# DemianMArin/HMM_Training

Measured on NVIDIA B200. Metric: baum_welch_frames_per_s_per_iter, higher is better.
Workload: dtype f64

## Files before the change

### hmm_training_b200/csrc/bw.cu

```cuda
#include <algorithm>
#include <cstdlib>
#include <functional>
#include <memory>
#include <numeric>

#include "bw_kernels.cuh"
#include "bwltr_kernels.cuh"

namespace hmmb {

__global__ void k_load_B(const double *__restrict__ B, int N, int M, double *__restrict__ Bt,
                         int32_t *__restrict__ b_has_zero) {
    const size_t w = blockIdx.y;
    for (int e = blockIdx.x * blockDim.x + threadIdx.x; e < N * M; e += gridDim.x * blockDim.x) {
        const int k = e / N, j = e - k * N;
        const double v = B[(w * N + j) * M + k];
        Bt[w * (size_t)M * N + e] = v > 0.0 ? v : 0.0;
        if (!(v > 0.0) && b_has_zero) b_has_zero[w] = 1;
    }
}
__global__ void k_load_clamped(const double *__restrict__ src, int64_t n, double *__restrict__ dst) {
    for (int64_t e = (int64_t)blockIdx.x * blockDim.x + threadIdx.x; e < n; e += (int64_t)gridDim.x * blockDim.x) {
        const double v = src[e];
        dst[e] = v > 0.0 ? v : 0.0;
// ... 1210 lines not shown
                s.d_word, s.d_foff, s.R, per_group, h->N, h->M, h->d_pi, h->d_A, h->d_Bt, h->d_spill, h->d_llseq,
                h->act_cur, h->d_flag);
    HMMB_TRY((launch_exact<SymT, false>(h)));
    HMMB_LAUNCH("bw_backward", (k_bw_bwdG<NP, SymT>), (unsigned)grid, BW_THREADS, 0, (const SymT *)s.d_obs, s.d_off, s.d_len,
                s.d_word, s.d_foff, s.R, per_group, h->N, h->M, h->d_A, h->d_Bt, h->d_spill, h->d_llseq, h->act_cur,
                h->d_accum, h->astride, h->d_flag, h->d_newflags);
    return HMMB_OK;
}

static int bwd4_warps(int M, int rep, bool bidiag, size_t smem_optin, size_t *smem) {
    int nw = bidiag ? BWD4_MAX_WARPS : 12;
    auto bytes = [&](int w) { return (size_t)M * rep * 4 * sizeof(double) + (size_t)w * M * 4 * sizeof(double) + (size_t)w * 4 * sizeof(double); };
    const size_t avail = smem_optin > 20 * 1024 ? smem_optin - 20 * 1024 : 0;
    while (nw > 1 && bytes(nw) > avail) --nw;
    *smem = bytes(nw);
    return nw;
}

template <bool BIDIAG, int MT, int REP>
static int launch_special_estep(hmmb_bw *h) {
    Ctx &c = ctx();
    SeqSet &s = h->s;
    if (s.ncta == 0) { s.pend.reset(); return HMMB_OK; }
    const size_t smem_f = (size_t)h->M * 5 * sizeof(double) + (size_t)((h->M + 15) & ~15);
    size_t smem_b = 0;
    const int bwd_threads = 32 * bwd4_warps(h->M, REP, BIDIAG, c.smem_optin, &smem_b);
    HMMB_CUDA(cudaFuncSetAttribute((k_bw_bwd4<BIDIAG, MT, REP>), cudaFuncAttributeMaxDynamicSharedMemorySize, (int)smem_b));
    const CtaWork *stage_work = s.ncta_fine > 0 ? s.d_work_fine : s.d_work;
    const int stage_ncta = s.ncta_fine > 0 ? s.ncta_fine : s.ncta;
    auto launch_range = [&](int c0, int c1) -> int {
        if (c1 <= c0) return HMMB_OK;
        HMMB_LAUNCH("bw_forward", k_bw_fwd4<BIDIAG>, (c1 - c0) * FWD4_SPLIT, BW_THREADS, smem_f, stage_work + c0, s.d_blks, (const uint4 *)s.d_obs,
                    s.d_len, h->d_pi, h->d_A, h->d_Bt, h->M, spill4(h), h->d_llseq, h->act_cur, h->d_flag,
                    h->d_allfull, FWD4_SPLIT, SYM_MASK);
        HMMB_LAUNCH("bw_backward", (k_bw_bwd4<BIDIAG, MT, REP>), c1 - c0, bwd_threads, smem_b, stage_work + c0, s.d_blks, (const uint4 *)s.d_obs,
                    s.d_len, h->d_A, h->d_Bt, h->M, spill4(h), h->d_llseq, h->act_cur, h->d_bzero,
                    h->d_allfull, h->d_partials + (size_t)c0 * h->pstride, h->pstride, h->d_flag, h->d_newflags);
        return HMMB_OK;
    };
    if (s.pend) {
        PendingPrepare &p = *s.pend;
        int bdone = 0, cdone = 0;
        cudaStream_t main_stream = c.stream;
        const bool side = p.nstage > 2;
        struct Restore { Ctx &c; cudaStream_t s; ~Restore() { c.stream = s; } } restore{c, main_stream};
        if (side) {
            cudaEvent_t fork = event_get();
            HMMB_CUDA(cudaEventRecord(fork, main_stream));
            for (auto st : c.stage_stream) HMMB_CUDA(cudaStreamWaitEvent(st, fork, 0));
            event_put(fork);
        }
        for (int j = 0; j < p.nstage; ++j) {
            if (side) c.stream = c.stage_stream[j & 1];
            HMMB_CUDA(cudaStreamWaitEvent(c.stream, p.up->ev[p.ev_index[j]], 0));
            HMMB_TRY(launch_repack_range(s, p.up->d_raw, p.idx_bytes, bdone, p.blk_end[j], s.d_bad));
            HMMB_TRY(launch_range(cdone, p.cta_end[j]));
            bdone = p.blk_end[j];
            cdone = p.cta_end[j];
        }
        c.stream = main_stream;
        if (side) {
            for (auto st : c.stage_stream) {
                cudaEvent_t join = event_get();
                HMMB_CUDA(cudaEventRecord(join, st));
                HMMB_CUDA(cudaStreamWaitEvent(main_stream, join, 0));
                event_put(join);
            }
        }
        h->check_bad = true;
        h->pend_release = std::move(s.pend);
        HMMB_TRY((launch_exact<uint16_t, true>(h)));
        HMMB_LAUNCH("bw_exact", k_bw_llstat_fix, stage_ncta, BW_THREADS, 0, stage_work, s.d_blks, h->d_llseq, h->act_cur,
                    h->d_flag, h->d_partials, h->pstride, h->M);
        h->estep_fine = s.ncta_fine > 0;
        return HMMB_OK;
    }
    h->estep_fine = false;
    HMMB_LAUNCH("bw_forward", k_bw_fwd4<BIDIAG>, (s.ncta_fwd ? s.ncta_fwd : s.ncta) * FWD4_SPLIT, BW_THREADS, smem_f,
                s.ncta_fwd ? s.d_work_fwd : s.d_work, s.d_blks, (const uint4 *)s.d_obs,
                s.d_len, h->d_pi, h->d_A, h->d_Bt, h->M, spill4(h), h->d_llseq, h->act_cur, h->d_flag,
                h->d_allfull, FWD4_SPLIT, SYM_MASK);
    HMMB_TRY((launch_exact<uint16_t, true>(h)));
    HMMB_LAUNCH("bw_backward", (k_bw_bwd4<BIDIAG, MT, REP>), s.ncta, bwd_threads, smem_b, s.d_work, s.d_blks, (const uint4 *)s.d_obs,
                s.d_len, h->d_A, h->d_Bt, h->M, spill4(h), h->d_llseq, h->act_cur, h->d_bzero,
                h->d_allfull, h->d_partials, h->pstride, h->d_flag, h->d_newflags);
    return HMMB_OK;
}

template <int NS>
static int launch_ltr_estep(hmmb_bw *h) {
    SeqSet &s = h->sl;
    if (s.ncta == 0) return HMMB_OK;
    const int M = h->M;
    const size_t smem_f = (size_t)M * NS * 8 + (size_t)M * 8 + (size_t)M * 2;
    const size_t smem_b = (size_t)M * NS * 8 + (size_t)LTR_WARPS * 32 * Ltr<NS>::ROWB + (size_t)2 * NS * 8 +
                          (size_t)LTR_WARPS * 2 * NS * 8;
    HMMB_CUDA(cudaFuncSetAttribute(k_bw_fwdL<NS>, cudaFuncAttributeMaxDynamicSharedMemorySize, (int)smem_f));
    HMMB_CUDA(cudaFuncSetAttribute(k_bw_bwdL<NS>, cudaFuncAttributeMaxDynamicSharedMemorySize, (int)smem_b));
    if (s.pend) {
        Ctx &c = ctx();
        PendingPrepare &p = *s.pend;
        int bdone = 0, cdone = 0;
        cudaStream_t main_stream = c.stream;
        const bool side = p.nstage > 2;
        struct Restore { Ctx &c; cudaStream_t s; ~Restore() { c.stream = s; } } restore{c, main_stream};
        if (side) {
            cudaEvent_t fork = event_get();
            HMMB_CUDA(cudaEventRecord(fork, main_stream));
            for (auto st : c.stage_stream) HMMB_CUDA(cudaStreamWaitEvent(st, fork, 0));
            event_put(fork);
        }
        for (int j = 0; j < p.nstage; ++j) {
            if (side) c.stream = c.stage_stream[j & 1];
            HMMB_CUDA(cudaStreamWaitEvent(c.stream, p.up->ev[p.ev_index[j]], 0));
// ... 504 lines not shown
```

### hmm_training_b200/csrc/bw4_kernels.cuh

```cuda
#pragma once

#include <type_traits>

#include "hmm_device.cuh"

namespace hmmb {

constexpr int BW_THREADS = 128;
constexpr int BW_WARPS = BW_THREADS / 32;
constexpr int SPC4 = 8;
constexpr unsigned SYM_MASK = 0x7ffu;
constexpr int SYM_BITS = 11;
constexpr int BW4_MAX_M = 512;
constexpr int BWD4_MAX_WARPS = 16;
constexpr int FWD4_SPLIT = 4;
constexpr int BWD4_REP = 8;

constexpr int REPACK_WARPS = 8;
__device__ __forceinline__ unsigned lanes_with_my_bit(unsigned sym, int bit) {
    int mine;
    asm("bfe.s32 %0, %1, %2, 1;" : "=r"(mine) : "r"(sym), "r"(bit));
    const unsigned set = __ballot_sync(0xffffffffu, mine != 0);
    return ~(set ^ (unsigned)mine);
}
// ... 81 lines not shown
    unsigned pmask;
};
__device__ __forceinline__ unsigned lut4(unsigned long long lut, unsigned m) {
    return (unsigned)(lut >> (m * 4u)) & 0xFu;
}
__device__ __forceinline__ Masks4 make_masks4(const double *__restrict__ Aw, const double *__restrict__ piw) {
    unsigned row[4];
#pragma unroll
    for (int i = 0; i < 4; ++i) {
        row[i] = 0u;
#pragma unroll
        for (int j = 0; j < 4; ++j) row[i] |= (__ldg(Aw + i * 4 + j) > 0.0) ? (1u << j) : 0u;
    }
    Masks4 mk;
    mk.lutF = mk.lutB = 0ull;
    for (unsigned m = 0; m < 16; ++m) {
        unsigned f = 0u, b = 0u;
#pragma unroll
        for (int i = 0; i < 4; ++i) {
            if ((m >> i) & 1u) f |= row[i];
            if (row[i] & m) b |= 1u << i;
        }
        mk.lutF |= (unsigned long long)f << (m * 4u);
        mk.lutB |= (unsigned long long)b << (m * 4u);
    }
    mk.pmask = 0u;
    if (piw) {
#pragma unroll
        for (int j = 0; j < 4; ++j) mk.pmask |= (__ldg(piw + j) > 0.0) ? (1u << j) : 0u;
    }
    return mk;
}
__device__ __forceinline__ double tiny_if(unsigned m, int j) { return __hiloint2double(0, (int)((m >> j) & 1u)); }

template <bool BIDIAG, bool SPILL, bool VECB = true, int REP = 1>
__device__ __forceinline__ double fwd4_run(int T, int tmax, const uint4 *__restrict__ op,
                                           const double2 *__restrict__ sB01, const double2 *__restrict__ sB23,
                                           const double *__restrict__ sBmax,
                                           const unsigned char *__restrict__ sBmask, const double *a,
                                           const double (&p)[4], double rmax, const Masks4 &mk,
                                           double2 *__restrict__ sp, bool &allfull, int slot = 0,
                                           unsigned symmask = SYM_MASK) {
    using S16 = Sym<uint16_t>;
    double al0 = 0.0, al1 = 0.0, al2 = 0.0, al3 = 0.0;
    double e0 = 0.0, e1 = 0.0, e2 = 0.0, e3 = 0.0;
    long long esum = 0;
    unsigned m = 0u;
    bool stop = false;
    bool allf = true;
    double ll = neg_inf();
    const double tiny = tiny_pos();
    const int nch = (tmax + SPC4 - 1) / SPC4;
    uint4 wnext = nch > 0 ? __ldg(op) : make_uint4(0, 0, 0, 0);
    for (int c = 0; c < nch; ++c) {
        uint4 w = wnext;
        if (c + 1 < nch) wnext = __ldg(op + (size_t)(c + 1) * 32);
#pragma unroll 2
        for (int s = 0; s < SPC4; ++s) {
            const int t = c * SPC4 + s;
            const unsigned sym = S16::pop_front(w) & symmask;
            if (t < T && !stop) {
                const double2 b01 = sB01[sym * REP + slot], b23 = sB23[sym * REP + slot];
                const unsigned r = (t == 0) ? mk.pmask : lut4(mk.lutF, m);
                m = r & (unsigned)sBmask[sym];
                double n0, n1, n2, n3, at0, at1, at2, at3;
                if (m == 0xFu && t > 0) {
                    if (BIDIAG) {
                        n0 = fma(al0, a[0], tiny);
                        n1 = fma(al1, a[1], fma(al0, a[4], tiny));
                        n2 = fma(al2, a[2], fma(al1, a[5], tiny));
                        n3 = fma(al3, a[3], fma(al2, a[6], tiny));
                    } else {
                        n0 = fma(al3, a[12], fma(al2, a[8], fma(al1, a[4], fma(al0, a[0], tiny))));
                        n1 = fma(al3, a[13], fma(al2, a[9], fma(al1, a[5], fma(al0, a[1], tiny))));
                        n2 = fma(al3, a[14], fma(al2, a[10], fma(al1, a[6], fma(al0, a[2], tiny))));
                        n3 = fma(al3, a[15], fma(al2, a[11], fma(al1, a[7], fma(al0, a[3], tiny))));
                    }
                    at0 = fma(n0, b01.x, tiny); at1 = fma(n1, b01.y, tiny);
                    at2 = fma(n2, b23.x, tiny); at3 = fma(n3, b23.y, tiny);
                } else if (m == 0u) {
                    stop = true;
                    n0 = n1 = n2 = n3 = at0 = at1 = at2 = at3 = 0.0;
                } else {
                    allf = allf && (m == 0xFu);
                    const double r0 = tiny_if(r, 0), r1 = tiny_if(r, 1), r2 = tiny_if(r, 2), r3 = tiny_if(r, 3);
                    if (t == 0) {
                        n0 = p[0]; n1 = p[1]; n2 = p[2]; n3 = p[3];
                    } else {
                        n0 = fma(al3, a_at<BIDIAG>(a, 3, 0), fma(al2, a_at<BIDIAG>(a, 2, 0), fma(al1, a_at<BIDIAG>(a, 1, 0), fma(al0, a_at<BIDIAG>(a, 0, 0), r0))));
                        n1 = fma(al3, a_at<BIDIAG>(a, 3, 1), fma(al2, a_at<BIDIAG>(a, 2, 1), fma(al1, a_at<BIDIAG>(a, 1, 1), fma(al0, a_at<BIDIAG>(a, 0, 1), r1))));
                        n2 = fma(al3, a_at<BIDIAG>(a, 3, 2), fma(al2, a_at<BIDIAG>(a, 2, 2), fma(al1, a_at<BIDIAG>(a, 1, 2), fma(al0, a_at<BIDIAG>(a, 0, 2), r2))));
                        n3 = fma(al3, a_at<BIDIAG>(a, 3, 3), fma(al2, a_at<BIDIAG>(a, 2, 3), fma(al1, a_at<BIDIAG>(a, 1, 3), fma(al0, a_at<BIDIAG>(a, 0, 3), r3))));
                    }
                    at0 = fma(n0, b01.x, tiny_if(m, 0)); at1 = fma(n1, b01.y, tiny_if(m, 1));
                    at2 = fma(n2, b23.x, tiny_if(m, 2)); at3 = fma(n3, b23.y, tiny_if(m, 3));
                }
                double ssum = (at0 + at1) + (at2 + at3);
                if (!stop && !(ssum >= TINY_STEP)) {
                    double o[4];
                    int Ex;
                    const int code = exact_products4(n0, n1, n2, n3, b01.x, b01.y, b23.x, b23.y, o, &Ex);
                    if (code == 0) {
                        stop = true;
                    } else if ((code == 2 && t > 0) || ((e0 + e1) + (e2 + e3)) > 0.0) {
                        stop = true;
                        ll = nan_mark();
                    } else {
                        esum += Ex;
                        at0 = o[0]; at1 = o[1]; at2 = o[2]; at3 = o[3];
                        ssum = (at0 + at1) + (at2 + at3);
                    }
                    allf = false;
                }
                if (!stop) {
                    const double sc = pow2_rescale(ssum, esum);
                    allf = allf && (__double2hiint(sc) >= 0x3ff00000);
                    al0 = at0 * sc; al1 = at1 * sc; al2 = at2 * sc; al3 = at3 * sc;
                    if (!VECB) {
                        e0 = fma(e0, rmax * sBmax[sym], 4.0 * ERR_UNIT) * sc;
                    } else {
                    double f0 = 0.0, f1 = 0.0, f2 = 0.0, f3 = 0.0;
                    if (t > 0) {
                        if (BIDIAG) {
                            f0 = e0 * a[0];
                            f1 = fma(e1, a[1], e0 * a[4]);
                            f2 = fma(e2, a[2], e1 * a[5]);
                            f3 = fma(e3, a[3], e2 * a[6]);
                        } else {
                            f0 = fma(e3, a[12], fma(e2, a[8], fma(e1, a[4], e0 * a[0])));
                            f1 = fma(e3, a[13], fma(e2, a[9], fma(e1, a[5], e0 * a[1])));
                            f2 = fma(e3, a[14], fma(e2, a[10], fma(e1, a[6], e0 * a[2])));
                            f3 = fma(e3, a[15], fma(e2, a[11], fma(e1, a[7], e0 * a[3])));
                        }
                    }
                    e0 = fma(f0, b01.x, ERR_UNIT) * sc;
                    e1 = fma(f1, b01.y, ERR_UNIT) * sc;
                    e2 = fma(f2, b23.x, ERR_UNIT) * sc;
                    e3 = fma(f3, b23.y, ERR_UNIT) * sc;
                    }
                    if (!(((e0 + e1) + (e2 + e3)) <= ERR_LIMIT)) {
                        stop = true;
                        ll = nan_mark();
                    }
                    if (t == T - 1 && !stop) ll = log((al0 + al1) + (al2 + al3)) + (double)esum * LN2;
                }
                if (SPILL && !stop) {
                    __stcs(sp + (size_t)t * 64, make_double2(al0, al1));
                    __stcs(sp + (size_t)t * 64 + 32, make_double2(al2, al3));
                }
            }
        }
    }
    allfull = allf && !stop;
    return ll;
}

template <bool BIDIAG, int REP>
__device__ __forceinline__ double score4_lean_run(int T, int tmax, const uint4 *__restrict__ op,
                                                  const double2 *__restrict__ b01row, const double2 *__restrict__ b23row,
                                                  const double *a, const double (&p)[4], const Masks4 &mk, int tstar,
                                                  bool &bad_out) {
    using S16 = Sym<uint16_t>;
    double al0 = 0.0, al1 = 0.0, al2 = 0.0, al3 = 0.0;
    int esum = 0;
    bool bad = false;
    unsigned m = 0u;
    auto step = [&](auto masked, int t, unsigned sym) {
        constexpr bool MASKED = decltype(masked)::value;
        const double2 b01 = b01row[sym * REP], b23 = b23row[sym * REP];
        double n0, n1, n2, n3;
        if (MASKED && t == 0) {
            n0 = p[0]; n1 = p[1]; n2 = p[2]; n3 = p[3];
        } else {
            matvec_fwd<BIDIAG>(a, al0, al1, al2, al3, n0, n1, n2, n3);
        }
        const double at0 = n0 * b01.x, at1 = n1 * b01.y, at2 = n2 * b23.x, at3 = n3 * b23.y;
        unsigned h0 = (unsigned)__double2hiint(at0), h1 = (unsigned)__double2hiint(at1);
        unsigned h2 = (unsigned)__double2hiint(at2), h3 = (unsigned)__double2hiint(at3);
        const unsigned hmax = max(max(h0, h1), max(h2, h3));
// ... 69 lines not shown
    const int tid = threadIdx.x;
    const double2 *src = reinterpret_cast<const double2 *>(Bt + (size_t)w * M * 4);
    double2 *dst = reinterpret_cast<double2 *>(sB);
    for (int e = tid; e < M; e += BW_THREADS) {
        const double2 x = __ldg(src + 2 * e), y = __ldg(src + 2 * e + 1);
        dst[e] = x;
        dst[M + e] = y;
        sBmax[e] = fmax(fmax(x.x, x.y), fmax(y.x, y.y));
        sBmask[e] = (unsigned char)((x.x > 0.0 ? 1 : 0) | (x.y > 0.0 ? 2 : 0) | (y.x > 0.0 ? 4 : 0) | (y.y > 0.0 ? 8 : 0));
    }
    load_Api4<BIDIAG>(pi, A, w, a, p, rmax, mk);
}

template <bool BIDIAG>
__device__ __forceinline__ void load_A4(const double *__restrict__ Aw, double *a) {
    if (BIDIAG) {
#pragma unroll
        for (int i = 0; i < 4; ++i) a[i] = __ldg(Aw + i * 5);
#pragma unroll
        for (int i = 0; i < 3; ++i) a[4 + i] = __ldg(Aw + i * 5 + 1);
    } else {
#pragma unroll
        for (int q = 0; q < 16; ++q) a[q] = __ldg(Aw + q);
    }
}

constexpr int FWD4_MIN_CTAS = 4;
template <bool BIDIAG>
__global__ void __launch_bounds__(BW_THREADS, FWD4_MIN_CTAS)
k_bw_fwd4(const CtaWork *__restrict__ work, const Blk *__restrict__ blks, const uint4 *__restrict__ obs_blk,
          const int32_t *__restrict__ len_sorted, const double *__restrict__ pi, const double *__restrict__ A,
          const double *__restrict__ Bt, int M, double2 *__restrict__ spill, double *__restrict__ ll_seq,
          const int32_t *__restrict__ active, uint8_t *__restrict__ flag, uint8_t *__restrict__ allfull, int split,
          unsigned symmask) {
    extern __shared__ double sB[];
    double *sBmax = sB + (size_t)M * 4;
    unsigned char *sBmask = reinterpret_cast<unsigned char *>(sBmax + M);
    CtaWork cw = work[blockIdx.x / split];
    if (!active[cw.word]) return;
    {
        const int nb = cw.blk_end - cw.blk_begin, part = blockIdx.x % split;
        const int lo = cw.blk_begin + (int)((int64_t)nb * part / split);
        cw.blk_end = cw.blk_begin + (int)((int64_t)nb * (part + 1) / split);
        cw.blk_begin = lo;
        if (cw.blk_begin >= cw.blk_end) return;
    }
    const int tid = threadIdx.x, lane = tid & 31, warp = tid >> 5;
    double a[BIDIAG ? 7 : 16], p[4], rmax;
    Masks4 mk;
    load_model4<BIDIAG>(pi, A, Bt, cw.word, M, sB, sBmax, sBmask, a, p, rmax, mk);
    __syncthreads();
    for (int b = cw.blk_begin + warp; b < cw.blk_end; b += BW_WARPS) {
        const Blk bk = blks[b];
        int T = lane < bk.nseq ? len_sorted[bk.first + lane] : 0;
        if (T > 0 && flag[bk.first + lane]) T = 0;
        bool af = false;
        const double ll = fwd4_run<BIDIAG, true>(T, bk.tmax, obs_blk + bk.obs_base + lane, reinterpret_cast<const double2 *>(sB),
                                                 reinterpret_cast<const double2 *>(sB) + M, sBmax, sBmask, a, p, rmax,
                                                 mk, spill + bk.spill_base * 64 + lane, af, 0, symmask);
        if (T > 0) {
            ll_seq[bk.first + lane] = ll;
            allfull[bk.first + lane] = af ? 1 : 0;
            if (ll != ll) raise_flag(flag, bk.first + lane);
        }
    }
}

__device__ __forceinline__ unsigned smem_u32(const void *p) { return (unsigned)__cvta_generic_to_shared(p); }
__device__ __forceinline__ unsigned hold32(unsigned x) { return __shfl_sync(0xffffffffu, x, threadIdx.x & 31); }
__device__ __forceinline__ double2 lds128_ro(unsigned addr) {
    double2 v;
    asm("ld.shared.v2.f64 {%0, %1}, [%2];" : "=d"(v.x), "=d"(v.y) : "r"(addr));
    return v;
}
__device__ __forceinline__ double2 lds128(unsigned addr) {
    double2 v;
    asm volatile("ld.shared.v2.f64 {%0, %1}, [%2];" : "=d"(v.x), "=d"(v.y) : "r"(addr) : "memory");
    return v;
}
__device__ __forceinline__ void sts128(unsigned addr, double2 v) {
    asm volatile("st.shared.v2.f64 [%0], {%1, %2};" ::"r"(addr), "d"(v.x), "d"(v.y) : "memory");
}
__device__ __forceinline__ double undef_f64() {
    double x;
    asm("" : "=d"(x));
    return x;
}
__device__ __forceinline__ void cnt_rmw4(unsigned row, unsigned off23, double g0, double g1, double g2, double g3) {
    double2 c01 = lds128(row), c23 = lds128(row + off23);
    c01.x += g0; c01.y += g1; c23.x += g2; c23.y += g3;
    sts128(row, c01); sts128(row + off23, c23);
}
__device__ __forceinline__ void cnt_round_sync() { __syncwarp(); }
__device__ __forceinline__ void cnt_update4(unsigned row, unsigned off23, bool act, int rank, double g0, double g1,
                                            double g2, double g3) {
    const int myrank = act ? rank : -1;
    const int maxrank = __reduce_max_sync(0xffffffffu, myrank);
    if (myrank == 0) cnt_rmw4(row, off23, g0, g1, g2, g3);
    if (maxrank > 0) {
        cnt_round_sync();
        if (myrank == 1) cnt_rmw4(row, off23, g0, g1, g2, g3);
#pragma unroll 1
        for (int r = 2; r <= maxrank; ++r) {
            cnt_round_sync();
            if (myrank == r) cnt_rmw4(row, off23, g0, g1, g2, g3);
        }
    }
    cnt_round_sync();
}

__device__ __forceinline__ bool all_pos4(double x0, double x1, double x2, double x3) {
    const unsigned m0 = (unsigned)__double2hiint(x0) | (unsigned)__double2loint(x0);
    const unsigned m1 = (unsigned)__double2hiint(x1) | (unsigned)__double2loint(x1);
    const unsigned m2 = (unsigned)__double2hiint(x2) | (unsigned)__double2loint(x2);
    const unsigned m3 = (unsigned)__double2hiint(x3) | (unsigned)__double2loint(x3);
    return min(min(m0, m1), min(m2, m3)) != 0u;
}
__device__ __forceinline__ double zero_to_tiny(double x) {
    const int hi = __double2hiint(x), lo = __double2loint(x);
    return __hiloint2double(hi, lo | (((hi | lo) == 0) ? 1 : 0));
}
__device__ __forceinline__ double pos_to_tiny(double x) {
    return __hiloint2double(0, ((__double2hiint(x) | __double2loint(x)) != 0) ? 1 : 0);
}
__device__ __forceinline__ void cp_async16(void *smem_dst, const void *gsrc) {
    asm volatile("cp.async.ca.shared.global [%0], [%1], 16;" ::"r"((unsigned)__cvta_generic_to_shared(smem_dst)), "l"(gsrc));
}
__device__ __forceinline__ void cp_async_commit() { asm volatile("cp.async.commit_group;" ::: "memory"); }
__device__ __forceinline__ void cp_async_wait_all() { asm volatile("cp.async.wait_group 0;" ::: "memory"); }
constexpr int BWD4_SPILL_PAD = 2;
constexpr int BWD_L2_PREFETCH = 12;
__device__ __forceinline__ void prefetch_l2(const void *p) { asm volatile("prefetch.global.L2 [%0];" ::"l"(p)); }
__device__ __forceinline__ void prefetch_l2_if(const void *p, bool on) {
    asm volatile("{\n\t.reg .pred pf;\n\tsetp.ne.u32 pf, %1, 0;\n\t@pf prefetch.global.L2 [%0];\n\t}" ::"l"(p), "r"((unsigned)on));
}
constexpr double LEAN_MIN = 0x1p-500;
constexpr unsigned LEAN_MIN_HI = (1023u - 500u) << 20;

__device__ __forceinline__ double recip_from_ref(double norm, double rref) {
    const double x = norm * rref;
    const int e = (__double2hiint(x) + 0x00040000) & 0x7ff00000;
    return __hiloint2double(__double2hiint(rref) - e + 0x3ff00000, __double2loint(rref));
}
constexpr double NORM_TOL = 1e-10;
constexpr unsigned NORM_TOL_HI = 0x3DDB7CDFu;
__device__ __forceinline__ bool norm_consistent(double norm, double r) {
    return ((unsigned)__double2hiint(fma(norm, r, -1.0)) & 0x7fffffffu) < NORM_TOL_HI;
}

template <bool BIDIAG>
struct Bwd4State {
    double v0, v1, v2, v3;
    double X[BIDIAG ? 7 : 16];
    double rref;
    unsigned seenX;
    bool imprecise;
    bool vpos;
};

template <bool BIDIAG>
__device__ __noinline__ void bwd4_step_slow(Bwd4State<BIDIAG> &st, const double *a, const double2 *__restrict__ sB01,
                                            const double2 *__restrict__ sB23,
                                            unsigned sym, bool last, double al0, double al1, double al2, double al3,
                                            double *g) {
    double v0 = st.v0, v1 = st.v1, v2 = st.v2, v3 = st.v3;
    double h0 = 1.0, h1 = 1.0, h2 = 1.0, h3 = 1.0;
    double w0 = 0.0, w1 = 0.0, w2 = 0.0, w3 = 0.0;
// ... 143 lines not shown
          const double2 *__restrict__ spill, const double *__restrict__ ll_seq, const int32_t *__restrict__ active,
          const int32_t *__restrict__ b_has_zero, const uint8_t *__restrict__ allfull, double *__restrict__ partials,
          int64_t pstride, uint8_t *__restrict__ flag, int32_t *__restrict__ new_flags) {
    using S16 = Sym<uint16_t>;
    const int M = MT ? MT : M_rt;
    const int nthreads = blockDim.x, nwarps = nthreads >> 5;
    extern __shared__ double smem[];
    double *sB = smem;
    double *sCnt = smem + (size_t)M * REP * 4;
    double *sPi = sCnt + (size_t)M * 4 * nwarps;
    __shared__ double sRed[BWD4_MAX_WARPS][20];
    __shared__ unsigned sSeen;
    __shared__ uint4 sW[2][BWD4_MAX_WARPS * 32];

    const CtaWork cw = work[blockIdx.x];
    double *part = partials + (size_t)blockIdx.x * pstride;
    const int tid = threadIdx.x, lane = tid & 31, warp = tid >> 5;
    if (!active[cw.word]) return;
    {
        const double2 *src = reinterpret_cast<const double2 *>(Bt + (size_t)cw.word * M * 4);
        double2 *dst01 = reinterpret_cast<double2 *>(sB), *dst23 = dst01 + (size_t)M * REP;
        for (int e = tid; e < M * REP; e += nthreads) {
            const int sym = e / REP;
            dst01[e] = __ldg(src + 2 * sym);
            dst23[e] = __ldg(src + 2 * sym + 1);
        }
        for (int e = tid; e < M * 4 * nwarps + nwarps * 4; e += nthreads) sCnt[e] = 0.0;
        if (tid == 0) sSeen = 0u;
    }
    double a[BIDIAG ? 7 : 16];
    load_A4<BIDIAG>(A + (size_t)cw.word * 16, a);
    const Masks4 mk = make_masks4(A + (size_t)cw.word * 16, nullptr);
    const bool lean_ok = (b_has_zero[cw.word] == 0) && (lut4(mk.lutB, 0xFu) == 0xFu);
    const double tiny = tiny_pos();
    __syncthreads();

    double2 *cntw01 = reinterpret_cast<double2 *>(sCnt + (size_t)warp * M * 4);
    const double2 *sB01 = reinterpret_cast<const double2 *>(sB) + (lane & (REP - 1)), *sB23 = sB01 + (size_t)M * REP;
    double *mypi = sPi + (size_t)warp * 4;
    const unsigned bbase = hold32(smem_u32(sB01)), cbase = hold32(smem_u32(cntw01));
    const unsigned B23_OFF = (unsigned)M * REP * 16u, CNT23_OFF = (unsigned)M * 16u;
    Bwd4State<BIDIAG> st;
#pragma unroll
    for (int q = 0; q < (BIDIAG ? 7 : 16); ++q) st.X[q] = 0.0;
    st.seenX = 0u;

    for (int b = cw.blk_begin + warp; b < cw.blk_end; b += nwarps) {
        const Blk bk = blks[b];
        int T = 0;
        bool apos = false;
        if (lane < bk.nseq) {
            T = len_sorted[bk.first + lane];
            if (!(ll_seq[bk.first + lane] > neg_inf())) T = 0;
            if (flag[bk.first + lane]) T = 0;
            apos = allfull[bk.first + lane] != 0;
        }
        st.v0 = st.v1 = st.v2 = st.v3 = 0.0;
        st.imprecise = false;
        st.vpos = false;
        st.rref = 1.0;
        const uint4 *op = obs_blk + bk.obs_base + lane;
        const double2 *sp = spill + bk.spill_base * 64 + lane;
        const int nch = (bk.tmax + SPC4 - 1) / SPC4;
        double2 P0_01 = make_double2(0.0, 0.0), P0_23 = P0_01, P1_01 = P0_01, P1_23 = P0_01;
        {
            const int r1 = nch * SPC4, r0 = max(r1 - BWD_L2_PREFETCH, 0);
            const char *base = reinterpret_cast<const char *>(sp - lane) + (size_t)r0 * 1024;
            for (int l = lane; l < (r1 - r0) * 8; l += 32) prefetch_l2(base + (size_t)l * 128);
            const int ta = bk.tmax - 1;
            if (ta < T) {
                const double2 x01 = __ldcs(sp + (size_t)ta * 64), x23 = __ldcs(sp + (size_t)ta * 64 + 32);
                if (ta & 1) { P1_01 = x01; P1_23 = x23; }
                else        { P0_01 = x01; P0_23 = x23; }
            }
        }
        int wbuf = 0;
        cp_async16(&sW[0][tid], op + (size_t)(nch - 1) * 32);
        cp_async_commit();

#define HMMB_BWD_STEP(T_, C_, O_, SP_, PACKED_)                                                                     \
    {                                                                                                               \
        const int t = (T_);                                                                                         \
        const double2 *spt = (SP_);          \
        const unsigned packed = (PACKED_);                                                                          \
        if (t < bk.tmax) {                                                                        \
            const unsigned sym = packed & SYM_MASK;                                                                 \
            const bool act = t < T;                                                                                 \
            const double al0 = P##C_##_01.x, al1 = P##C_##_01.y, al2 = P##C_##_23.x, al3 = P##C_##_23.y;            \
             \
             \
             \
             \
            P##O_##_01 = __ldcs(spt - 64);                                                                          \
            P##O_##_23 = __ldcs(spt - 64 + 32);                                                                     \
            const unsigned brow = bbase + sym * (unsigned)(REP * 16);                                               \
            const unsigned crow = cbase + sym * 16u;                                                                \
            const int rank = (int)(packed >> SYM_BITS);                                                             \
            double g0 = undef_f64(), g1 = undef_f64(), g2 = undef_f64(), g3 = undef_f64();                          \
            if (act) {                                                                                              \
                bool done = false;                                                                                  \
                if (lean_ok && st.vpos) {              \
                        \
                       \
                        \
                    double q0, q1, q2, q3;                                                                          \
                    if (BIDIAG) {                                                                                   \
                        q0 = fma(a[4], st.v1, fma(a[0], st.v0, tiny));                                              \
                        q1 = fma(a[5], st.v2, fma(a[1], st.v1, tiny));                                              \
                        q2 = fma(a[6], st.v3, fma(a[2], st.v2, tiny));                                              \
                        q3 = fma(a[3], st.v3, tiny);                                                                \
                    } else {                                                                                        \
                        q0 = fma(a[3], st.v3, fma(a[2], st.v2, fma(a[1], st.v1, fma(a[0], st.v0, tiny))));          \
                        q1 = fma(a[7], st.v3, fma(a[6], st.v2, fma(a[5], st.v1, fma(a[4], st.v0, tiny))));          \
                        q2 = fma(a[11], st.v3, fma(a[10], st.v2, fma(a[9], st.v1, fma(a[8], st.v0, tiny))));        \
                        q3 = fma(a[15], st.v3, fma(a[14], st.v2, fma(a[13], st.v1, fma(a[12], st.v0, tiny))));      \
                    }                                                                                               \
                    const double qs = (q0 + q1) + (q2 + q3);                                                        \
                    const double c0 = al0 * q0, c1 = al1 * q1, c2 = al2 * q2, c3 = al3 * q3;                        \
                    const double norm = (c0 + c1) + (c2 + c3);                                                      \
                    const double r = recip_from_ref(norm, st.rref);                \
                                   \
                    const unsigned lo2 = min((unsigned)__double2hiint(norm), (unsigned)__double2hiint(qs));         \
                    if ((lo2 >= LEAN_MIN_HI) & norm_consistent(norm, r) && (apos || all_pos4(al0, al1, al2, al3))) {\
                                 \
                        g0 = fma(c0, r, tiny); g1 = fma(c1, r, tiny); g2 = fma(c2, r, tiny); g3 = fma(c3, r, tiny); \
                        const double u0 = al0 * r, u1 = al1 * r, u2 = al2 * r, u3 = al3 * r;                        \
                        if (BIDIAG) {                                                                               \
                            st.X[0] = fma(u0, st.v0, st.X[0]); st.X[1] = fma(u1, st.v1, st.X[1]);                   \
                            st.X[2] = fma(u2, st.v2, st.X[2]); st.X[3] = fma(u3, st.v3, st.X[3]);                   \
                            st.X[4] = fma(u0, st.v1, st.X[4]); st.X[5] = fma(u1, st.v2, st.X[5]);                   \
                            st.X[6] = fma(u2, st.v3, st.X[6]);                                                      \
                        } else {                                                                                    \
                            st.X[0] = fma(u0, st.v0, st.X[0]);   st.X[1] = fma(u0, st.v1, st.X[1]);                 \
                            st.X[2] = fma(u0, st.v2, st.X[2]);   st.X[3] = fma(u0, st.v3, st.X[3]);                 \
                            st.X[4] = fma(u1, st.v0, st.X[4]);   st.X[5] = fma(u1, st.v1, st.X[5]);                 \
                            st.X[6] = fma(u1, st.v2, st.X[6]);   st.X[7] = fma(u1, st.v3, st.X[7]);                 \
                            st.X[8] = fma(u2, st.v0, st.X[8]);   st.X[9] = fma(u2, st.v1, st.X[9]);                 \
                            st.X[10] = fma(u2, st.v2, st.X[10]); st.X[11] = fma(u2, st.v3, st.X[11]);               \
                            st.X[12] = fma(u3, st.v0, st.X[12]); st.X[13] = fma(u3, st.v1, st.X[13]);               \
                            st.X[14] = fma(u3, st.v2, st.X[14]); st.X[15] = fma(u3, st.v3, st.X[15]);               \
                        }                                                                                           \
                        st.seenX = 0xffffu;                                \
                        const double sc = pow2_rescale_noacc(qs);                                                   \
                        const double h0 = q0 * sc, h1 = q1 * sc, h2 = q2 * sc, h3 = q3 * sc;        \
                        const double2 b01 = lds128_ro(brow), b23 = lds128_ro(brow + B23_OFF);                       \
                        st.v0 = fma(b01.x, h0, tiny); st.v1 = fma(b01.y, h1, tiny);                                 \
                        st.v2 = fma(b23.x, h2, tiny); st.v3 = fma(b23.y, h3, tiny);                                 \
                        const double vs = (st.v0 + st.v1) + (st.v2 + st.v3);                                        \
                        if ((unsigned)__double2hiint(vs) < LEAN_MIN_HI) {      \
                            double vv[4];                                                                           \
                             \
                            if (bwd4_v_slow(zero_to_tiny(h0), zero_to_tiny(h1), zero_to_tiny(h2), zero_to_tiny(h3), b01.x, b01.y,       \
                                            b23.x, b23.y, vv)) st.imprecise = true;   \
                            st.v0 = vv[0]; st.v1 = vv[1]; st.v2 = vv[2]; st.v3 = vv[3];                             \
                            st.vpos = all_pos4(vv[0], vv[1], vv[2], vv[3]);                                         \
                        }                                                                                           \
                        done = true;                                                                                \
                    }                                                                                               \
                }                                                                                                   \
                if (!done) {                                                                                        \
                    if (t == T - 1) {                                                                               \
                        \
                        \
                        \
                        const double n0 = (al0 + al1) + (al2 + al3);   \
                        const double r0 = 1.0 / n0;                                                                 \
                        st.rref = r0;                                                                               \
                        g0 = fma(al0, r0, pos_to_tiny(al0)); g1 = fma(al1, r0, pos_to_tiny(al1));                   \
                        g2 = fma(al2, r0, pos_to_tiny(al2)); g3 = fma(al3, r0, pos_to_tiny(al3));                   \
                        const double2 b01 = lds128_ro(brow), b23 = lds128_ro(brow + B23_OFF);                       \
                        st.v0 = b01.x; st.v1 = b01.y; st.v2 = b23.x; st.v3 = b23.y;                                 \
                        st.vpos = all_pos4(b01.x, b01.y, b23.x, b23.y);                                             \
                    } else {                                                                                        \
                              \
                             \
                        Bwd4State<BIDIAG> tmp = st;                                                                 \
                        double g[4];                                                                                \
                        bwd4_step_slow<BIDIAG>(tmp, a, sB01, sB23, sym * REP, false, al0, al1, al2, al3, g);        \
                        st = tmp;                                                                                   \
                        g0 = g[0]; g1 = g[1]; g2 = g[2]; g3 = g[3];                                                 \
                    }                                                                                               \
                }                                                                                                   \
            }                                                                                                       \
            if (t == 0) {  \
                const int am = act ? -1 : 0;          \
                double p0 = __hiloint2double(__double2hiint(g0) & am, __double2loint(g0) & am);                     \
                double p1 = __hiloint2double(__double2hiint(g1) & am, __double2loint(g1) & am);                     \
                double p2 = __hiloint2double(__double2hiint(g2) & am, __double2loint(g2) & am);                     \
                double p3 = __hiloint2double(__double2hiint(g3) & am, __double2loint(g3) & am);                     \
                _Pragma("unroll") for (int o = 16; o > 0; o >>= 1) {                                                \
                    p0 += __shfl_xor_sync(0xffffffffu, p0, o); p1 += __shfl_xor_sync(0xffffffffu, p1, o);           \
                    p2 += __shfl_xor_sync(0xffffffffu, p2, o); p3 += __shfl_xor_sync(0xffffffffu, p3, o);           \
                }                                                                                                   \
                if (lane == 0) { mypi[0] += p0; mypi[1] += p1; mypi[2] += p2; mypi[3] += p3; }                      \
            }                                                                                                       \
                            \
            cnt_update4(crow, CNT23_OFF, act, rank, g0, g1, g2, g3);                                                \
        }                                                                                                           \
    }

        const double2 *spp = sp + (size_t)(nch * SPC4 - 2) * 64;
        for (int c = nch - 1; c >= 0; --c) {
            cp_async_wait_all();
            uint4 w = sW[wbuf][tid];
            wbuf ^= 1;
            if (c > 0) {
                cp_async16(&sW[wbuf][tid], op + (size_t)(c - 1) * 32);
                cp_async_commit();
            }
#pragma unroll 1
            for (int pr = SPC4 / 2 - 1; pr >= 0; --pr) {
                if (c * SPC4 + 2 * pr >= BWD_L2_PREFETCH && lane < 16)
                    prefetch_l2(reinterpret_cast<const char *>(spp) - BWD_L2_PREFETCH * 1024 + lane * (128 - 16));
                const unsigned p1 = S16::pop_back(w);
                HMMB_BWD_STEP(c * SPC4 + 2 * pr + 1, 1, 0, spp + 64, p1)
                const unsigned p0 = S16::pop_back(w);
                HMMB_BWD_STEP(c * SPC4 + 2 * pr, 0, 1, spp, p0)
                spp -= 2 * 64;
            }
        }
#undef HMMB_BWD_STEP
        if (st.imprecise) {
            raise_flag(flag, bk.first + lane);
            atomicAdd(new_flags, 1);
        }
    }

    double Xf[16];
    if (BIDIAG) {
#pragma unroll
        for (int q = 0; q < 16; ++q) Xf[q] = 0.0;
        Xf[0] = st.X[0]; Xf[5] = st.X[1]; Xf[10] = st.X[2]; Xf[15] = st.X[3];
        Xf[1] = st.X[4]; Xf[6] = st.X[5]; Xf[11] = st.X[6];
    } else {
#pragma unroll
        for (int q = 0; q < 16; ++q) Xf[q] = st.X[q];
    }
#pragma unroll
    for (int q = 0; q < 16; ++q) {
        double v = Xf[q];
#pragma unroll
        for (int o = 16; o > 0; o >>= 1) v += __shfl_xor_sync(0xffffffffu, v, o);
        if (lane == 0) sRed[warp][4 + q] = v;
    }
    if (lane == 0) {
#pragma unroll
        for (int q = 0; q < 4; ++q) sRed[warp][q] = mypi[q];
    }
    const unsigned seenW = __reduce_or_sync(0xffffffffu, st.seenX);
    if (lane == 0) atomicOr(&sSeen, seenW);
// ... 26 lines not shown
```

Before: 65.62 billion.

## Skip spilling odd-step alphas and recompute them in the backward pass

For words with no zero emissions and a fully connected forward mask, the forward kernel now skips storing odd-timestep alpha vectors to the spill buffer when the step needs no underflow handling. The backward kernel rebuilds each odd alpha from the preceding even alpha with one lean forward step, and falls back to a predicated load only for lanes where the value was actually stored. This halves the spill write and read traffic in the common case, at the cost of extra FMA work and warp-vote branching in the backward loop. The recomputation has to reproduce the forward-pass rounding bit-for-bit for correctness to hold.

```diff
diff --git a/hmm_training_b200/csrc/bw.cu b/hmm_training_b200/csrc/bw.cu
--- a/hmm_training_b200/csrc/bw.cu
+++ b/hmm_training_b200/csrc/bw.cu
@@ -1266,7 +1266,7 @@
         if (c1 <= c0) return HMMB_OK;
         HMMB_LAUNCH("bw_forward", k_bw_fwd4<BIDIAG>, (c1 - c0) * FWD4_SPLIT, BW_THREADS, smem_f, stage_work + c0, s.d_blks, (const uint4 *)s.d_obs,
                     s.d_len, h->d_pi, h->d_A, h->d_Bt, h->M, spill4(h), h->d_llseq, h->act_cur, h->d_flag,
-                    h->d_allfull, FWD4_SPLIT, SYM_MASK);
+                    h->d_allfull, FWD4_SPLIT, SYM_MASK, h->d_bzero);
         HMMB_LAUNCH("bw_backward", (k_bw_bwd4<BIDIAG, MT, REP>), c1 - c0, bwd_threads, smem_b, stage_work + c0, s.d_blks, (const uint4 *)s.d_obs,
                     s.d_len, h->d_A, h->d_Bt, h->M, spill4(h), h->d_llseq, h->act_cur, h->d_bzero,
                     h->d_allfull, h->d_partials + (size_t)c0 * h->pstride, h->pstride, h->d_flag, h->d_newflags);
@@ -1313,7 +1313,7 @@
     HMMB_LAUNCH("bw_forward", k_bw_fwd4<BIDIAG>, (s.ncta_fwd ? s.ncta_fwd : s.ncta) * FWD4_SPLIT, BW_THREADS, smem_f,
                 s.ncta_fwd ? s.d_work_fwd : s.d_work, s.d_blks, (const uint4 *)s.d_obs,
                 s.d_len, h->d_pi, h->d_A, h->d_Bt, h->M, spill4(h), h->d_llseq, h->act_cur, h->d_flag,
-                h->d_allfull, FWD4_SPLIT, SYM_MASK);
+                h->d_allfull, FWD4_SPLIT, SYM_MASK, h->d_bzero);
     HMMB_TRY((launch_exact<uint16_t, true>(h)));
     HMMB_LAUNCH("bw_backward", (k_bw_bwd4<BIDIAG, MT, REP>), s.ncta, bwd_threads, smem_b, s.d_work, s.d_blks, (const uint4 *)s.d_obs,
                 s.d_len, h->d_A, h->d_Bt, h->M, spill4(h), h->d_llseq, h->act_cur, h->d_bzero,
diff --git a/hmm_training_b200/csrc/bw4_kernels.cuh b/hmm_training_b200/csrc/bw4_kernels.cuh
--- a/hmm_training_b200/csrc/bw4_kernels.cuh
+++ b/hmm_training_b200/csrc/bw4_kernels.cuh
@@ -137,6 +137,42 @@
     return mk;
 }
 __device__ __forceinline__ double tiny_if(unsigned m, int j) { return __hiloint2double(0, (int)((m >> j) & 1u)); }
+__device__ __forceinline__ bool all_pos4(double x0, double x1, double x2, double x3) {
+    const unsigned m0 = (unsigned)__double2hiint(x0) | (unsigned)__double2loint(x0);
+    const unsigned m1 = (unsigned)__double2hiint(x1) | (unsigned)__double2loint(x1);
+    const unsigned m2 = (unsigned)__double2hiint(x2) | (unsigned)__double2loint(x2);
+    const unsigned m3 = (unsigned)__double2hiint(x3) | (unsigned)__double2loint(x3);
+    return min(min(m0, m1), min(m2, m3)) != 0u;
+}
+
+template <bool BIDIAG>
+__device__ __forceinline__ void lean_at4(const double *a, double al0, double al1, double al2, double al3, double2 b01,
+                                         double2 b23, double tiny, double &n0, double &n1, double &n2, double &n3,
+                                         double &at0, double &at1, double &at2, double &at3) {
+    if (BIDIAG) {
+        n0 = fma(al0, a[0], tiny);
+        n1 = fma(al1, a[1], fma(al0, a[4], tiny));
+        n2 = fma(al2, a[2], fma(al1, a[5], tiny));
+        n3 = fma(al3, a[3], fma(al2, a[6], tiny));
+    } else {
+        n0 = fma(al3, a[12], fma(al2, a[8], fma(al1, a[4], fma(al0, a[0], tiny))));
+        n1 = fma(al3, a[13], fma(al2, a[9], fma(al1, a[5], fma(al0, a[1], tiny))));
+        n2 = fma(al3, a[14], fma(al2, a[10], fma(al1, a[6], fma(al0, a[2], tiny))));
+        n3 = fma(al3, a[15], fma(al2, a[11], fma(al1, a[7], fma(al0, a[3], tiny))));
+    }
+    at0 = fma(n0, b01.x, tiny); at1 = fma(n1, b01.y, tiny);
+    at2 = fma(n2, b23.x, tiny); at3 = fma(n3, b23.y, tiny);
+}
+__device__ __forceinline__ double step_sum4(double at0, double at1, double at2, double at3) {
+    return (at0 + at1) + (at2 + at3);
+}
+__device__ __forceinline__ void rescale4(double sc, double at0, double at1, double at2, double at3, double &al0,
+                                         double &al1, double &al2, double &al3) {
+    al0 = __dmul_rn(at0, sc); al1 = __dmul_rn(at1, sc); al2 = __dmul_rn(at2, sc); al3 = __dmul_rn(at3, sc);
+}
+__device__ __forceinline__ bool lean_skip4(bool lean_word, double al0, double al1, double al2, double al3, double ssum) {
+    return lean_word && all_pos4(al0, al1, al2, al3) && ssum >= TINY_STEP;
+}
 
 template <bool BIDIAG, bool SPILL, bool VECB = true, int REP = 1>
 __device__ __forceinline__ double fwd4_run(int T, int tmax, const uint4 *__restrict__ op,
@@ -145,7 +181,7 @@
                                            const unsigned char *__restrict__ sBmask, const double *a,
                                            const double (&p)[4], double rmax, const Masks4 &mk,
                                            double2 *__restrict__ sp, bool &allfull, int slot = 0,
-                                           unsigned symmask = SYM_MASK) {
+                                           unsigned symmask = SYM_MASK, bool lean_word = false) {
     using S16 = Sym<uint16_t>;
     double al0 = 0.0, al1 = 0.0, al2 = 0.0, al3 = 0.0;
     double e0 = 0.0, e1 = 0.0, e2 = 0.0, e3 = 0.0;
@@ -170,19 +206,7 @@
                 m = r & (unsigned)sBmask[sym];
                 double n0, n1, n2, n3, at0, at1, at2, at3;
                 if (m == 0xFu && t > 0) {
-                    if (BIDIAG) {
-                        n0 = fma(al0, a[0], tiny);
-                        n1 = fma(al1, a[1], fma(al0, a[4], tiny));
-                        n2 = fma(al2, a[2], fma(al1, a[5], tiny));
-                        n3 = fma(al3, a[3], fma(al2, a[6], tiny));
-                    } else {
-                        n0 = fma(al3, a[12], fma(al2, a[8], fma(al1, a[4], fma(al0, a[0], tiny))));
-                        n1 = fma(al3, a[13], fma(al2, a[9], fma(al1, a[5], fma(al0, a[1], tiny))));
-                        n2 = fma(al3, a[14], fma(al2, a[10], fma(al1, a[6], fma(al0, a[2], tiny))));
-                        n3 = fma(al3, a[15], fma(al2, a[11], fma(al1, a[7], fma(al0, a[3], tiny))));
-                    }
-                    at0 = fma(n0, b01.x, tiny); at1 = fma(n1, b01.y, tiny);
-                    at2 = fma(n2, b23.x, tiny); at3 = fma(n3, b23.y, tiny);
+                    lean_at4<BIDIAG>(a, al0, al1, al2, al3, b01, b23, tiny, n0, n1, n2, n3, at0, at1, at2, at3);
                 } else if (m == 0u) {
                     stop = true;
                     n0 = n1 = n2 = n3 = at0 = at1 = at2 = at3 = 0.0;
@@ -200,7 +224,8 @@
                     at0 = fma(n0, b01.x, tiny_if(m, 0)); at1 = fma(n1, b01.y, tiny_if(m, 1));
                     at2 = fma(n2, b23.x, tiny_if(m, 2)); at3 = fma(n3, b23.y, tiny_if(m, 3));
                 }
-                double ssum = (at0 + at1) + (at2 + at3);
+                double ssum = step_sum4(at0, at1, at2, at3);
+                const bool skip = SPILL && (t & 1) && lean_skip4(lean_word, al0, al1, al2, al3, ssum);
                 if (!stop && !(ssum >= TINY_STEP)) {
                     double o[4];
                     int Ex;
@@ -213,14 +238,14 @@
                     } else {
                         esum += Ex;
                         at0 = o[0]; at1 = o[1]; at2 = o[2]; at3 = o[3];
-                        ssum = (at0 + at1) + (at2 + at3);
+                        ssum = step_sum4(at0, at1, at2, at3);
                     }
                     allf = false;
                 }
                 if (!stop) {
                     const double sc = pow2_rescale(ssum, esum);
                     allf = allf && (__double2hiint(sc) >= 0x3ff00000);
-                    al0 = at0 * sc; al1 = at1 * sc; al2 = at2 * sc; al3 = at3 * sc;
+                    rescale4(sc, at0, at1, at2, at3, al0, al1, al2, al3);
                     if (!VECB) {
                         e0 = fma(e0, rmax * sBmax[sym], 4.0 * ERR_UNIT) * sc;
                     } else {
@@ -249,7 +274,7 @@
                     }
                     if (t == T - 1 && !stop) ll = log((al0 + al1) + (al2 + al3)) + (double)esum * LN2;
                 }
-                if (SPILL && !stop) {
+                if (SPILL && !stop && !skip) {
                     __stcs(sp + (size_t)t * 64, make_double2(al0, al1));
                     __stcs(sp + (size_t)t * 64 + 32, make_double2(al2, al3));
                 }
@@ -385,7 +410,7 @@
           const int32_t *__restrict__ len_sorted, const double *__restrict__ pi, const double *__restrict__ A,
           const double *__restrict__ Bt, int M, double2 *__restrict__ spill, double *__restrict__ ll_seq,
           const int32_t *__restrict__ active, uint8_t *__restrict__ flag, uint8_t *__restrict__ allfull, int split,
-          unsigned symmask) {
+          unsigned symmask, const int32_t *__restrict__ b_has_zero) {
     extern __shared__ double sB[];
     double *sBmax = sB + (size_t)M * 4;
     unsigned char *sBmask = reinterpret_cast<unsigned char *>(sBmax + M);
@@ -402,6 +427,7 @@
     double a[BIDIAG ? 7 : 16], p[4], rmax;
     Masks4 mk;
     load_model4<BIDIAG>(pi, A, Bt, cw.word, M, sB, sBmax, sBmask, a, p, rmax, mk);
+    const bool lean_word = (b_has_zero[cw.word] == 0) && (lut4(mk.lutF, 0xFu) == 0xFu);
     __syncthreads();
     for (int b = cw.blk_begin + warp; b < cw.blk_end; b += BW_WARPS) {
         const Blk bk = blks[b];
@@ -410,7 +436,7 @@
         bool af = false;
         const double ll = fwd4_run<BIDIAG, true>(T, bk.tmax, obs_blk + bk.obs_base + lane, reinterpret_cast<const double2 *>(sB),
                                                  reinterpret_cast<const double2 *>(sB) + M, sBmax, sBmask, a, p, rmax,
-                                                 mk, spill + bk.spill_base * 64 + lane, af, 0, symmask);
+                                                 mk, spill + bk.spill_base * 64 + lane, af, 0, symmask, lean_word);
         if (T > 0) {
             ll_seq[bk.first + lane] = ll;
             allfull[bk.first + lane] = af ? 1 : 0;
@@ -462,13 +488,6 @@
     cnt_round_sync();
 }
 
-__device__ __forceinline__ bool all_pos4(double x0, double x1, double x2, double x3) {
-    const unsigned m0 = (unsigned)__double2hiint(x0) | (unsigned)__double2loint(x0);
-    const unsigned m1 = (unsigned)__double2hiint(x1) | (unsigned)__double2loint(x1);
-    const unsigned m2 = (unsigned)__double2hiint(x2) | (unsigned)__double2loint(x2);
-    const unsigned m3 = (unsigned)__double2hiint(x3) | (unsigned)__double2loint(x3);
-    return min(min(m0, m1), min(m2, m3)) != 0u;
-}
 __device__ __forceinline__ double zero_to_tiny(double x) {
     const int hi = __double2hiint(x), lo = __double2loint(x);
     return __hiloint2double(hi, lo | (((hi | lo) == 0) ? 1 : 0));
@@ -486,6 +505,11 @@
 __device__ __forceinline__ void prefetch_l2(const void *p) { asm volatile("prefetch.global.L2 [%0];" ::"l"(p)); }
 __device__ __forceinline__ void prefetch_l2_if(const void *p, bool on) {
     asm volatile("{\n\t.reg .pred pf;\n\tsetp.ne.u32 pf, %1, 0;\n\t@pf prefetch.global.L2 [%0];\n\t}" ::"l"(p), "r"((unsigned)on));
+}
+__device__ __forceinline__ void ldcs_if(const double2 *p, bool on, double2 &v) {
+    asm("{\n\t.reg .pred q;\n\t.reg .u64 g;\n\tsetp.ne.u32 q, %3, 0;\n\tcvta.to.global.u64 g, %2;\n\t"
+        "@q ld.global.cs.v2.f64 {%0, %1}, [g];\n\t}"
+        : "+d"(v.x), "+d"(v.y) : "l"(p), "r"((unsigned)on));
 }
 constexpr double LEAN_MIN = 0x1p-500;
 constexpr unsigned LEAN_MIN_HI = (1023u - 500u) << 20;
@@ -695,6 +719,7 @@
     load_A4<BIDIAG>(A + (size_t)cw.word * 16, a);
     const Masks4 mk = make_masks4(A + (size_t)cw.word * 16, nullptr);
     const bool lean_ok = (b_has_zero[cw.word] == 0) && (lut4(mk.lutB, 0xFu) == 0xFu);
+    const bool lean_word = (b_has_zero[cw.word] == 0) && (lut4(mk.lutF, 0xFu) == 0xFu);
     const double tiny = tiny_pos();
     __syncthreads();
 
@@ -725,38 +750,26 @@
         const uint4 *op = obs_blk + bk.obs_base + lane;
         const double2 *sp = spill + bk.spill_base * 64 + lane;
         const int nch = (bk.tmax + SPC4 - 1) / SPC4;
-        double2 P0_01 = make_double2(0.0, 0.0), P0_23 = P0_01, P1_01 = P0_01, P1_23 = P0_01;
+        double2 PE_01 = make_double2(0.0, 0.0), PE_23 = PE_01, PO_01 = PE_01, PO_23 = PE_01, PN_01, PN_23;
         {
             const int r1 = nch * SPC4, r0 = max(r1 - BWD_L2_PREFETCH, 0);
             const char *base = reinterpret_cast<const char *>(sp - lane) + (size_t)r0 * 1024;
-            for (int l = lane; l < (r1 - r0) * 8; l += 32) prefetch_l2(base + (size_t)l * 128);
-            const int ta = bk.tmax - 1;
-            if (ta < T) {
-                const double2 x01 = __ldcs(sp + (size_t)ta * 64), x23 = __ldcs(sp + (size_t)ta * 64 + 32);
-                if (ta & 1) { P1_01 = x01; P1_23 = x23; }
-                else        { P0_01 = x01; P0_23 = x23; }
-            }
+            for (int l = lane; l < (r1 - r0) * 4; l += 32) prefetch_l2(base + (size_t)(l >> 3) * 2048 + (l & 7) * 128);
+            const int te = (bk.tmax - 1) & ~1;
+            if (te < T) { PE_01 = __ldcs(sp + (size_t)te * 64); PE_23 = __ldcs(sp + (size_t)te * 64 + 32); }
         }
         int wbuf = 0;
         cp_async16(&sW[0][tid], op + (size_t)(nch - 1) * 32);
         cp_async_commit();
 
-#define HMMB_BWD_STEP(T_, C_, O_, SP_, PACKED_)                                                                     \
+#define HMMB_BWD_STEP(T_, P_, PACKED_, B01_, B23_)                                                                  \
     {                                                                                                               \
         const int t = (T_);                                                                                         \
-        const double2 *spt = (SP_);          \
         const unsigned packed = (PACKED_);                                                                          \
-        if (t < bk.tmax) {                                                                        \
+        {                                                                                                           \
             const unsigned sym = packed & SYM_MASK;                                                                 \
             const bool act = t < T;                                                                                 \
-            const double al0 = P##C_##_01.x, al1 = P##C_##_01.y, al2 = P##C_##_23.x, al3 = P##C_##_23.y;            \
-             \
-             \
-             \
-             \
-            P##O_##_01 = __ldcs(spt - 64);                                                                          \
-            P##O_##_23 = __ldcs(spt - 64 + 32);                                                                     \
-            const unsigned brow = bbase + sym * (unsigned)(REP * 16);                                               \
+            const double al0 = P_##_01.x, al1 = P_##_01.y, al2 = P_##_23.x, al3 = P_##_23.y;                        \
             const unsigned crow = cbase + sym * 16u;                                                                \
             const int rank = (int)(packed >> SYM_BITS);                                                             \
             double g0 = undef_f64(), g1 = undef_f64(), g2 = undef_f64(), g3 = undef_f64();                          \
@@ -806,7 +819,7 @@
                         st.seenX = 0xffffu;                                \
                         const double sc = pow2_rescale_noacc(qs);                                                   \
                         const double h0 = q0 * sc, h1 = q1 * sc, h2 = q2 * sc, h3 = q3 * sc;        \
-                        const double2 b01 = lds128_ro(brow), b23 = lds128_ro(brow + B23_OFF);                       \
+                        const double2 b01 = (B01_), b23 = (B23_);                                                   \
                         st.v0 = fma(b01.x, h0, tiny); st.v1 = fma(b01.y, h1, tiny);                                 \
                         st.v2 = fma(b23.x, h2, tiny); st.v3 = fma(b23.y, h3, tiny);                                 \
                         const double vs = (st.v0 + st.v1) + (st.v2 + st.v3);                                        \
@@ -831,7 +844,7 @@
                         st.rref = r0;                                                                               \
                         g0 = fma(al0, r0, pos_to_tiny(al0)); g1 = fma(al1, r0, pos_to_tiny(al1));                   \
                         g2 = fma(al2, r0, pos_to_tiny(al2)); g3 = fma(al3, r0, pos_to_tiny(al3));                   \
-                        const double2 b01 = lds128_ro(brow), b23 = lds128_ro(brow + B23_OFF);                       \
+                        const double2 b01 = (B01_), b23 = (B23_);                                                   \
                         st.v0 = b01.x; st.v1 = b01.y; st.v2 = b23.x; st.v3 = b23.y;                                 \
                         st.vpos = all_pos4(b01.x, b01.y, b23.x, b23.y);                                             \
                     } else {                                                                                        \
@@ -873,12 +886,34 @@
             }
 #pragma unroll 1
             for (int pr = SPC4 / 2 - 1; pr >= 0; --pr) {
-                if (c * SPC4 + 2 * pr >= BWD_L2_PREFETCH && lane < 16)
+                const int te = c * SPC4 + 2 * pr;
+                if (te >= BWD_L2_PREFETCH && lane < 8)
                     prefetch_l2(reinterpret_cast<const char *>(spp) - BWD_L2_PREFETCH * 1024 + lane * (128 - 16));
                 const unsigned p1 = S16::pop_back(w);
-                HMMB_BWD_STEP(c * SPC4 + 2 * pr + 1, 1, 0, spp + 64, p1)
                 const unsigned p0 = S16::pop_back(w);
-                HMMB_BWD_STEP(c * SPC4 + 2 * pr, 0, 1, spp, p0)
+                if (te < bk.tmax) {
+                    if (te + 1 < bk.tmax) {
+                        const unsigned bro = bbase + (p1 & SYM_MASK) * (unsigned)(REP * 16);
+                        const double2 bo01 = lds128_ro(bro), bo23 = lds128_ro(bro + B23_OFF);
+                        double n0, n1, n2, n3, at0, at1, at2, at3;
+                        lean_at4<BIDIAG>(a, PE_01.x, PE_01.y, PE_23.x, PE_23.y, bo01, bo23, tiny, n0, n1, n2, n3, at0,
+                                         at1, at2, at3);
+                        const double ssum = step_sum4(at0, at1, at2, at3);
+                        const bool skip = lean_skip4(lean_word, PE_01.x, PE_01.y, PE_23.x, PE_23.y, ssum);
+                        rescale4(pow2_rescale_noacc(ssum), at0, at1, at2, at3, PO_01.x, PO_01.y, PO_23.x, PO_23.y);
+                        const bool stored = !skip && te + 1 < T;
+                        if (__any_sync(0xffffffffu, stored)) {
+                            ldcs_if(spp + 64, stored, PO_01);
+                            ldcs_if(spp + 64 + 32, stored, PO_23);
+                        }
+                        HMMB_BWD_STEP(te + 1, PO, p1, bo01, bo23)
+                    }
+                    PN_01 = __ldcs(spp - 2 * 64);
+                    PN_23 = __ldcs(spp - 2 * 64 + 32);
+                    const unsigned bre = bbase + (p0 & SYM_MASK) * (unsigned)(REP * 16);
+                    HMMB_BWD_STEP(te, PE, p0, lds128_ro(bre), lds128_ro(bre + B23_OFF))
+                    PE_01 = PN_01; PE_23 = PN_23;
+                }
                 spp -= 2 * 64;
             }
         }
```

After: 66.98 billion (median of 6 runs). 1.02x the previous value.
